# colmap/glomap

Hardware: NVIDIA H100
Metric: observations/sec per BA LM-iteration (higher is better)
Workload: dtype f64

## Files before the change

### glomap_b200/csrc/ba_kernels.cuh

```cuda
#pragma once
#include "common.cuh"
#include "pcg.cuh"

namespace b200 {

constexpr int kCamRec = 8;
constexpr int kIntrRec = 8;
constexpr double kZEps = 1e-12;
constexpr int kSeg = 256;
__host__ __device__ constexpr int seg_split(int n) { return n <= 0 ? 0 : (n < kSeg + kSeg / 2 ? 1 : (n + kSeg / 2) / kSeg); }
constexpr int kIntrSmem = 16;
constexpr int kJpDoubles = 6;
constexpr int kSensorRec = 16;

struct BAView {
  int C, P, K;
  long long N;
  int n_tiles;
  int n_segs;
  int min_views;
  const int* obs_cam;
  const int* obs_pt;
  const double2* obs_xy;
  const unsigned* pt_begin;
// ... 401 lines not shown
      sm.red[5][tid] = o.Jp[2] * o.Jp[2] + o.Jp[5] * o.Jp[5];
      sm.red[6][tid] = o.Jp[0] * o.r[0] + o.Jp[3] * o.r[1];
      sm.red[7][tid] = o.Jp[1] * o.r[0] + o.Jp[4] * o.r[1];
      sm.red[8][tid] = o.Jp[2] * o.r[0] + o.Jp[5] * o.r[1];
      fence_proxy_async_smem();
      __syncthreads();
      if (tid == 0) {
        if (V2) tma_store_1d(v.W + (size_t)(o0 + c0) * kJpDoubles, sm.Wt, (uint32_t)nc * kJpDoubles * 8);
        else tma_store_1d(v.W + (size_t)(o0 + c0) * kWDoubles, sm.Wt, (uint32_t)nc * kWBytes);
        tma_store_commit();
      }
      for (int item = tid; item < npts * 9; item += kTile) {
        const int j = item / 9, k = item - 9 * j;
        const int lo = max((int)sm.pb[j] - (int)(o0 + c0), 0), hi = min((int)sm.pb[j + 1] - (int)(o0 + c0), nc);
        double a = 0.0;
        for (int i = lo; i < hi; ++i) a += sm.red[k][i];
        sm.acc[k][j] += a;
      }
      if (tid == 0) tma_store_wait_read();
      __syncthreads();
    }
  }
  double gmax = 0.0;
  if (points_var && tid < npts) {
    const size_t p = (size_t)(p0 + tid);
    if (pvalid) {
#pragma unroll
      for (int k = 0; k < 6; ++k) v.V[6 * p + k] = sm.acc[k][tid];
#pragma unroll
      for (int k = 0; k < 3; ++k) {
        const double gk = sm.acc[6 + k][tid];
        v.gp[3 * p + k] = gk;
        gmax = fmax(gmax, fabs(gk));
      }
    } else {
#pragma unroll
      for (int k = 0; k < 6; ++k) v.V[6 * p + k] = 0.0;
#pragma unroll
      for (int k = 0; k < 3; ++k) v.gp[3 * p + k] = 0.0;
    }
  }
  cost = block_sum(cost, sm.scratch);
  if (tid == 0 && cost != 0.0) atomicAdd(&scal[0], cost);
  gmax = block_max(gmax, sm.scratch);
  if (tid == 0 && gmax > 0.0) atomic_max_nonneg(&scal[1], gmax);
}

__global__ void __launch_bounds__(128) ba_linearize_cams(BAView v, const double* __restrict__ cam_rec,
                                                        const double* __restrict__ intr_rec,
                                                        const double* __restrict__ points, double huber_a) {
  const int warp = (blockIdx.x * blockDim.x + threadIdx.x) >> 5;
  const int lane = threadIdx.x & 31;
  if (warp >= v.n_segs) return;
  const int cam = v.seg_cam[warp];
  const int b = v.seg_begin[warp], e = v.seg_end[warp];
  const double4 q4c = *reinterpret_cast<const double4*>(cam_rec + (size_t)cam * kCamRec);
  const double4 t4c = *reinterpret_cast<const double4*>(cam_rec + (size_t)cam * kCamRec + 4);
  const double* irc = intr_rec + (size_t)v.seg_intr[warp] * kIntrRec;
  const double* src = sensor_of_seg(v, warp);
  double U[21], g[6];
#pragma unroll
  for (int k = 0; k < 21; ++k) U[k] = 0.0;
#pragma unroll
  for (int k = 0; k < 6; ++k) g[k] = 0.0;
  for (int i = b + lane; i < e; i += 32) {
    const int pt = v.pt_c[i];
    const double2 xy = v.xy_c[i];
    const double X0 = points[3 * (size_t)pt], X1 = points[3 * (size_t)pt + 1], X2 = points[3 * (size_t)pt + 2];
    ObsLin o;
    linearize_obs(q4c, t4c, irc, src, X0, X1, X2, xy, huber_a, o);
    double Jc[2][6];
#pragma unroll
    for (int a = 0; a < 2; ++a)
#pragma unroll
      for (int k = 0; k < 3; ++k) {
        Jc[a][k] = o.Jr[3 * a + k];
        Jc[a][3 + k] = o.Jt[3 * a + k];
      }
    int idx = 0;
#pragma unroll
    for (int i2 = 0; i2 < 6; ++i2) {
#pragma unroll
      for (int j = i2; j < 6; ++j) U[idx++] += Jc[0][i2] * Jc[0][j] + Jc[1][i2] * Jc[1][j];
      g[i2] += Jc[0][i2] * o.r[0] + Jc[1][i2] * o.r[1];
    }
  }
#pragma unroll
  for (int k = 0; k < 21; ++k) {
    const double s = warp_sum(U[k]);
    if (lane == k && s != 0.0) atomicAdd(&v.U[(size_t)cam * 21 + k], s);
  }
#pragma unroll
  for (int k = 0; k < 6; ++k) {
    const double s = warp_sum(g[k]);
    if (lane == 21 + k && s != 0.0) atomicAdd(&v.gc[(size_t)cam * 6 + k], s);
  }
}

__global__ void ba_finalize_cams(int C, double* __restrict__ U, double* __restrict__ gc,
                                 const unsigned char* __restrict__ cam_mask, double* __restrict__ jscale_c,
                                 int set_jscale, double* __restrict__ scal, const double* __restrict__ gslots, int nslots) {
  const int c = blockIdx.x * blockDim.x + threadIdx.x;
  double gmax = 0.0;
  if (blockIdx.x == 0 && threadIdx.x < nslots) gmax = gslots[threadIdx.x];
  if (c < C) {
    const int mask = cam_mask[c];
#pragma unroll
    for (int i = 0; i < 6; ++i) {
      const int di = sym_idx(6, i, i);
      const bool fixed = (i < 3) ? (mask & 1) : (mask & 2);
      double d = U[(size_t)c * 21 + di];
      if (fixed || !(d > 0.0)) {
        for (int j = 0; j < 6; ++j) U[(size_t)c * 21 + (i <= j ? sym_idx(6, i, j) : sym_idx(6, j, i))] = 0.0;
        U[(size_t)c * 21 + di] = 1.0;
        gc[(size_t)c * 6 + i] = 0.0;
        if (set_jscale) jscale_c[(size_t)c * 6 + i] = -1.0;
      } else {
        if (set_jscale) jscale_c[(size_t)c * 6 + i] = 1.0 / (1.0 + sqrt(d));
        gmax = fmax(gmax, fabs(gc[(size_t)c * 6 + i]));
      }
    }
  }
  gmax = warp_max(gmax);
  if ((threadIdx.x & 31) == 0 && gmax > 0.0) atomic_max_nonneg(&scal[1], gmax);
}

__global__ void ba_damp_cams(int C, const double* __restrict__ U, const double* __restrict__ jscale_c, double radius,
                             double* __restrict__ Dc) {
  const int i = blockIdx.x * blockDim.x + threadIdx.x;
  if (i >= C * 6) return;
  const int c = i / 6, k = i % 6;
  const double js = jscale_c[i];
  if (js < 0.0) {
    Dc[i] = 0.0;
    return;
  }
  const double d = U[(size_t)c * 21 + sym_idx(6, k, k)];
  const double js2 = js * js;
  Dc[i] = fmin(fmax(d * js2, 1e-6), 1e32) / (radius * js2);
}

__device__ __forceinline__ void point_damping(const double* V6, const double* js, double radius, double Dp[3]) {
  const double d[3] = {V6[0], V6[3], V6[5]};
#pragma unroll
  for (int k = 0; k < 3; ++k) {
    const double js2 = js[k] * js[k];
    Dp[k] = fmin(fmax(d[k] * js2, 1e-6), 1e32) / (radius * js2);
  }
}
__global__ void ba_damp_points(int P, const double* __restrict__ V, double* __restrict__ jscale_p, int set_jscale,
                               double radius, double* __restrict__ Vinv) {
  const int p = blockIdx.x * blockDim.x + threadIdx.x;
  if (p >= P) return;
  double v6[6];
#pragma unroll
  for (int k = 0; k < 6; ++k) v6[k] = V[6 * (size_t)p + k];
  double js[3];
  if (set_jscale) {
    js[0] = 1.0 / (1.0 + sqrt(v6[0]));
    js[1] = 1.0 / (1.0 + sqrt(v6[3]));
    js[2] = 1.0 / (1.0 + sqrt(v6[5]));
#pragma unroll
    for (int k = 0; k < 3; ++k) jscale_p[3 * (size_t)p + k] = js[k];
  } else {
#pragma unroll
    for (int k = 0; k < 3; ++k) js[k] = jscale_p[3 * (size_t)p + k];
  }
  double Dp[3];
  point_damping(v6, js, radius, Dp);
  v6[0] += Dp[0];
  v6[3] += Dp[1];
  v6[5] += Dp[2];
  double inv[6];
  sym3_inverse(v6, inv);
#pragma unroll
  for (int k = 0; k < 6; ++k) Vinv[6 * (size_t)p + k] = inv[k];
}

__global__ void __launch_bounds__(128) ba_schur_diag(BAView v) {
  const int warp = (blockIdx.x * blockDim.x + threadIdx.x) >> 5;
  const int lane = threadIdx.x & 31;
  if (warp >= v.n_segs) return;
  const int cam = v.seg_cam[warp];
  const int b = v.seg_begin[warp], e = v.seg_end[warp];
  double S[21];
#pragma unroll
  for (int k = 0; k < 21; ++k) S[k] = 0.0;
  for (int i = b + lane; i < e; i += 32) {
    const int o = v.camord_obs[i];
    const int pt = v.pt_c[i];
    double w[18], vi[6];
    const double2* wp = reinterpret_cast<const double2*>(v.W + (size_t)o * kWDoubles);
#pragma unroll
    for (int k = 0; k < 9; ++k) {
      const double2 t = wp[k];
      w[2 * k] = t.x;
      w[2 * k + 1] = t.y;
    }
    const double2* vp = reinterpret_cast<const double2*>(v.Vinv + (size_t)pt * 6);
#pragma unroll
    for (int k = 0; k < 3; ++k) {
      const double2 t = vp[k];
      vi[2 * k] = t.x;
      vi[2 * k + 1] = t.y;
    }
    double T[6][3];
#pragma unroll
    for (int r = 0; r < 6; ++r) sym3_mul(vi, &w[3 * r], T[r]);
    int idx = 0;
#pragma unroll
    for (int r = 0; r < 6; ++r)
#pragma unroll
      for (int c = r; c < 6; ++c)
        S[idx++] += T[r][0] * w[3 * c] + T[r][1] * w[3 * c + 1] + T[r][2] * w[3 * c + 2];
  }
#pragma unroll
  for (int k = 0; k < 21; ++k) {
    const double s = warp_sum(S[k]);
    if (lane == k && s != 0.0) atomicAdd(&v.Sd[(size_t)cam * 21 + k], s);
  }
}

__global__ void ba_build_precond(int C, const double* __restrict__ U, const double* __restrict__ Dc,
                                 const double* __restrict__ Sd, double* __restrict__ Minv) {
  const int c = blockIdx.x * blockDim.x + threadIdx.x;
  if (c >= C) return;
  double m[21];
#pragma unroll
  for (int k = 0; k < 21; ++k) m[k] = U[(size_t)c * 21 + k] - (Sd ? Sd[(size_t)c * 21 + k] : 0.0);
#pragma unroll
  for (int i = 0; i < 6; ++i) m[sym_idx(6, i, i)] += Dc[(size_t)c * 6 + i];
  double inv[21];
  spd_inverse_packed<6>(m, inv);
#pragma unroll
  for (int k = 0; k < 21; ++k) Minv[(size_t)c * 21 + k] = inv[k];
}

struct K3Smem {
  alignas(128) double Wt[kTile * kWDoubles];
  double t[3][kTile + 1];
  double z[3][kTilePts + 1];
  unsigned pb[kTilePts + 1];
  double scratch[32];
  alignas(8) uint64_t mbar;
};

template <int MODE>
__global__ void __launch_bounds__(kTile, B200_K3_MIN_CTAS) ba_schur_pass(BAView v, const double* __restrict__ x, double* __restrict__ y,
                                                          const double* __restrict__ points,
                                                          double* __restrict__ points_new, double radius,
                                                          double* __restrict__ bscal, const double* __restrict__ spk = nullptr,
                                                          const double* __restrict__ dk = nullptr, int m_intr = 0,
                                                          const PcgCtl* __restrict__ ctl = nullptr) {
  extern __shared__ __align__(128) unsigned char smem_raw[];
  if (ctl && ctl->done) return;
  K3Smem& sm = *reinterpret_cast<K3Smem*>(smem_raw);
  const int tile = blockIdx.x;
  const int tid = threadIdx.x;
  const int4 td = v.tile_desc[tile];
  const int p0 = td.x, npts = td.y, n = td.w;
  const unsigned o0 = (unsigned)td.z, o1 = o0 + (unsigned)n;
  const int nchunks = (n + kTile - 1) / kTile;
  if (tid == 0) {
    mbar_init(&sm.mbar, 1);
    fence_mbar_init();
    if (MODE != 1 && n > 0) {
      const int nc0 = min(kTile, n);
      mbar_arrive_expect_tx(&sm.mbar, (uint32_t)nc0 * kWBytes);
      tma_load_1d(sm.Wt, v.W + (size_t)o0 * kWDoubles, (uint32_t)nc0 * kWBytes, &sm.mbar);
    }
  }
  int cam_pf = 0, pt_pf = 0;
  double2 xa_pf = make_double2(0, 0), xb_pf = xa_pf, xc_pf = xa_pf;
  if (MODE != 1 && tid < n) {
    cam_pf = v.obs_cam[o0 + tid];
    if (MODE == 0) pt_pf = v.obs_pt[o0 + tid];
    const double2* xp = reinterpret_cast<const double2*>(x + (size_t)cam_pf * 6);
    xa_pf = xp[0];
    xb_pf = xp[1];
    xc_pf = xp[2];
  }
  if (tid < npts) {
    sm.pb[tid] = v.pt_begin[p0 + tid];
    if (tid == npts - 1) sm.pb[npts] = o1;
    sm.z[0][tid] = sm.z[1][tid] = sm.z[2][tid] = 0.0;
  }
  __syncthreads();
  uint32_t phase = 0;
  if (MODE != 1) {
    for (int ch = 0; ch < nchunks; ++ch) {
      const int c0 = ch * kTile;
      const int nc = min(kTile, n - c0);
      if (tid == 0 && ch > 0) {
        mbar_arrive_expect_tx(&sm.mbar, (uint32_t)nc * kWBytes);
        tma_load_1d(sm.Wt, v.W + (size_t)(o0 + c0) * kWDoubles, (uint32_t)nc * kWBytes, &sm.mbar);
      }
      double xc[6] = {0, 0, 0, 0, 0, 0};
      const bool active = tid < nc;
      if (active) {
        if (ch > 0) {
          cam_pf = v.obs_cam[o0 + c0 + tid];
          const double2* xp = reinterpret_cast<const double2*>(x + (size_t)cam_pf * 6);
          xa_pf = xp[0];
          xb_pf = xp[1];
          xc_pf = xp[2];
        }
        xc[0] = xa_pf.x; xc[1] = xa_pf.y; xc[2] = xb_pf.x; xc[3] = xb_pf.y; xc[4] = xc_pf.x; xc[5] = xc_pf.y;
      }
      mbar_wait(&sm.mbar, phase);
      phase ^= 1;
      double t0 = 0, t1 = 0, t2 = 0;
      if (active) {
        const double2* wr = reinterpret_cast<const double2*>(sm.Wt + tid * kWDoubles);
#pragma unroll
        for (int r = 0; r < 6; r += 2) {
          const double2 q0 = wr[(3 * r) / 2], q1 = wr[(3 * r) / 2 + 1], q2 = wr[(3 * r) / 2 + 2];
          t0 += q0.x * xc[r] + q1.y * xc[r + 1];
          t1 += q0.y * xc[r] + q2.x * xc[r + 1];
          t2 += q1.x * xc[r] + q2.y * xc[r + 1];
        }
      }
      sm.t[0][tid] = t0;
      sm.t[1][tid] = t1;
      sm.t[2][tid] = t2;
      __syncthreads();
      for (int item = tid; item < npts * 3; item += kTile) {
        const int j = item / 3, k = item - 3 * j;
        const int lo = max((int)sm.pb[j] - (int)(o0 + c0), 0), hi = min((int)sm.pb[j + 1] - (int)(o0 + c0), nc);
        double a = 0.0;
// ... 254 lines not shown
```

### glomap_b200/csrc/ba_kernels_v3.cuh

```cuda
#pragma once
#include "ba_kernels_v2.cuh"

namespace b200 {

constexpr int kEllWindow = 1024;
constexpr int kEllThreads = 128;

struct EllView {
  int n_groups;
  const int* row0;
  const int* pt;
  const int* len;
  const int* cam;
  const double2* xy;
  const unsigned short* sensor;
  double* A;
  double* B = nullptr;
};

template <class Sort>
__global__ void __launch_bounds__(kEllWindow) ell_sort_window(int P, int min_views, const unsigned* __restrict__ pt_begin,
                                                              int* __restrict__ ell_pt, int* __restrict__ ell_len,
                                                              int* __restrict__ ell_slot, int* __restrict__ group_rows) {
  __shared__ typename Sort::TempStorage tmp;
  const int t = threadIdx.x;
  const int p = blockIdx.x * kEllWindow + t;
  int len = -1;
  if (p < P) {
    len = (int)(pt_begin[p + 1] - pt_begin[p]);
    if (len < min_views) len = 0;
  }
  unsigned key[1] = {p < P ? (unsigned)(0xffffff - min(len, 0xffffff)) : 0xffffffffu};
  int val[1] = {t};
  Sort(tmp).Sort(key, val, 0, 25);
  const int src = blockIdx.x * kEllWindow + val[0];
  const int slot = blockIdx.x * kEllWindow + t;
  const bool real = key[0] != 0xffffffffu;
  const int l = real ? (int)(0xffffff - key[0]) : 0;
  ell_pt[slot] = real ? src : -1;
  ell_len[slot] = l;
  if (real) ell_slot[src] = slot;
  if ((t & 31) == 0) group_rows[slot >> 5] = l;
}

__global__ void ell_scatter_obs(long long N, int min_views, const int* __restrict__ obs_pt, const unsigned* __restrict__ pt_begin,
                                const int* __restrict__ obs_cam, const double2* __restrict__ obs_xy,
                                const unsigned short* __restrict__ obs_sensor, const int* __restrict__ ell_slot,
                                const int* __restrict__ row0, int* __restrict__ ell_cam, double2* __restrict__ ell_xy,
                                unsigned short* __restrict__ ell_sensor) {
  const long long o = (long long)blockIdx.x * blockDim.x + threadIdx.x;
  if (o >= N) return;
  const int p = obs_pt[o];
  const unsigned b = pt_begin[p];
  if ((int)(pt_begin[p + 1] - b) < min_views) return;
  const int slot = ell_slot[p];
  const size_t dst = ((size_t)row0[slot >> 5] + (size_t)(o - b)) * 32 + (slot & 31);
  ell_cam[dst] = obs_cam[o];
  ell_xy[dst] = obs_xy[o];
  if (obs_sensor) ell_sensor[dst] = obs_sensor[o];
}

template <int NK>
__global__ void __launch_bounds__(kEllThreads, NK > 0 ? 3 : B200_E1_MIN_CTAS) ba3_linearize_points(BAView v, EllView ell,
                                                                               const double* __restrict__ cam_rec,
                                                                               const double* __restrict__ intr_rec,
                                                                               const double* __restrict__ points,
                                                                               double huber_a, int points_var,
                                                                               double* __restrict__ part_cost,
                                                                               double* __restrict__ part_gmax,
                                                                               const IntrVarRec* __restrict__ ivar) {
  const int slot = blockIdx.x * kEllThreads + threadIdx.x;
  const int lane = threadIdx.x & 31;
  const int g = slot >> 5;
  double cost = 0.0, gmax = 0.0;
  if (g < ell.n_groups) {
    const int pt = ell.pt[slot];
    const int mylen = ell.len[slot];
    const int r0 = ell.row0[g], nrow = ell.row0[g + 1] - r0;
    double X0 = 0, X1 = 0, X2 = 0;
    if (pt >= 0) {
      X0 = points[3 * (size_t)pt]; X1 = points[3 * (size_t)pt + 1]; X2 = points[3 * (size_t)pt + 2];
    }
    double V[6] = {0, 0, 0, 0, 0, 0}, gp[3] = {0, 0, 0};
#if B200_E1_PIPE
    int camB = 0;
    double2 xyA = make_double2(0, 0), xyB = xyA;
    double4 qA = make_double4(0, 0, 0, 1), tA = make_double4(0, 0, 0, 0);
    if (mylen > 0) {
      const size_t i0 = (size_t)r0 * 32 + lane;
      const int camA = ld_stream(ell.cam + i0);
      xyA = ld_stream(ell.xy + i0);
      if (mylen > 1) {
        camB = ld_stream(ell.cam + i0 + 32);
        xyB = ld_stream(ell.xy + i0 + 32);
      }
      qA = ld_rec32(cam_rec + (size_t)camA * kCamRec);
      tA = ld_rec32(cam_rec + (size_t)camA * kCamRec + 4);
    }
#if B200_E1_PIPE >= 2
    double4 qB2 = qA, tB2 = tA;
    int camC2 = 0;
    if (mylen > 1) {
      qB2 = ld_rec32(cam_rec + (size_t)camB * kCamRec);
      tB2 = ld_rec32(cam_rec + (size_t)camB * kCamRec + 4);
    }
    if (mylen > 2) camC2 = ld_stream(ell.cam + (size_t)r0 * 32 + lane + 64);
#endif
    for (int j = 0; j < nrow; ++j) {
      if (j >= mylen) break;
      const size_t idx = ((size_t)r0 + j) * 32 + lane;
#if B200_E1_PIPE >= 2
      double4 qB = qB2, tB = tB2;
      double4 qC = qB2, tC = tB2;
      int camC = 0, camD = 0;
      double2 xyC = xyB;
      if (j + 2 < mylen) {
        qC = ld_rec32(cam_rec + (size_t)camC2 * kCamRec);
        tC = ld_rec32(cam_rec + (size_t)camC2 * kCamRec + 4);
        xyC = ld_stream(ell.xy + idx + 64);
      }
      if (j + 3 < mylen) camD = ld_stream(ell.cam + idx + 96);
      (void)camC;
#else
      double4 qB = qA, tB = tA;
      int camC = 0;
      double2 xyC = xyB;
      if (j + 1 < mylen) {
        qB = ld_rec32(cam_rec + (size_t)camB * kCamRec);
        tB = ld_rec32(cam_rec + (size_t)camB * kCamRec + 4);
      }
      if (j + 2 < mylen) {
        camC = ld_stream(ell.cam + idx + 64);
        xyC = ld_stream(ell.xy + idx + 64);
      }
#endif
      const double* sr = ell.sensor ? v.sensor_rec + (size_t)ell.sensor[idx] * kSensorRec : nullptr;
      const int blk = obs_intr_idx(tA, sr);
      const double* ir = intr_rec + (size_t)blk * kIntrRec;
      ObsCore o;
      obs_core(qA, tA, ir, sr, X0, X1, X2, xyA, huber_a, o);
      cost += 0.5 * o.rho0;
      if (points_var) {
        double Jp[6], A[6], b[3];
        obs_point_blocks(o, Jp, A, b);
        double* row = ell.A + ((size_t)r0 + j) * (6 * 32) + lane;
#pragma unroll
        for (int k = 0; k < 6; ++k) {
          st_stream(row + 32 * k, A[k]);
          V[k] += A[k];
        }
        gp[0] += b[0]; gp[1] += b[1]; gp[2] += b[2];
        if (NK > 0) {
          constexpr int NKK = NK > 0 ? NK : 1;
          double Jk[2][NKK], Bo[3 * NKK];
          obs_intr_rows<NK>(o, ld_intr(ir), ivar[blk], Jp, Jk, Bo);
          double* rowB = ell.B + ((size_t)r0 + j) * (3 * NK * 32) + lane;
#pragma unroll
          for (int k = 0; k < 3 * NK; ++k) st_stream(rowB + 32 * k, Bo[k]);
        }
      }
#if B200_E1_PIPE >= 2
      qA = qB; tA = tB; qB2 = qC; tB2 = tC; xyA = xyB; xyB = xyC; camC2 = camD;
#else
      qA = qB; tA = tB; xyA = xyB; xyB = xyC; camB = camC;
#endif
    }
#else
#pragma unroll 2
    for (int j = 0; j < nrow; ++j) {
      if (j >= mylen) continue;
      const size_t idx = ((size_t)r0 + j) * 32 + lane;
      const int cam = ld_stream(ell.cam + idx);
      const double2 xy = ld_stream(ell.xy + idx);
      const double4 q4 = ld_rec32(cam_rec + (size_t)cam * kCamRec);
      const double4 t4 = ld_rec32(cam_rec + (size_t)cam * kCamRec + 4);
      const double* sr = ell.sensor ? v.sensor_rec + (size_t)ell.sensor[idx] * kSensorRec : nullptr;
      const int blk = obs_intr_idx(t4, sr);
      const double* ir = intr_rec + (size_t)blk * kIntrRec;
      ObsCore o;
      obs_core(q4, t4, ir, sr, X0, X1, X2, xy, huber_a, o);
      cost += 0.5 * o.rho0;
      if (points_var) {
        double Jp[6], A[6], b[3];
        obs_point_blocks(o, Jp, A, b);
        double* row = ell.A + ((size_t)r0 + j) * (6 * 32) + lane;
#pragma unroll
        for (int k = 0; k < 6; ++k) {
          st_stream(row + 32 * k, A[k]);
          V[k] += A[k];
        }
        gp[0] += b[0]; gp[1] += b[1]; gp[2] += b[2];
        if (NK > 0) {
          constexpr int NKK = NK > 0 ? NK : 1;
          double Jk[2][NKK], Bo[3 * NKK];
          obs_intr_rows<NK>(o, ld_intr(ir), ivar[blk], Jp, Jk, Bo);
          double* rowB = ell.B + ((size_t)r0 + j) * (3 * NK * 32) + lane;
#pragma unroll
          for (int k = 0; k < 3 * NK; ++k) st_stream(rowB + 32 * k, Bo[k]);
        }
      }
    }
#endif
    if (points_var && pt >= 0) {
#pragma unroll
      for (int k = 0; k < 6; ++k) v.V[6 * (size_t)pt + k] = V[k];
#pragma unroll
      for (int k = 0; k < 3; ++k) {
        v.gp[3 * (size_t)pt + k] = gp[k];
        gmax = fmax(gmax, fabs(gp[k]));
      }
    }
  }
  cost = warp_sum(cost);
  gmax = warp_max(gmax);
  if (lane == 0) {
    part_cost[slot >> 5] = cost;
    part_gmax[slot >> 5] = gmax;
  }
}

__global__ void __launch_bounds__(kEllThreads) ba3_cost(BAView v, EllView ell, const double* __restrict__ cam_rec,
                                                         const double* __restrict__ intr_rec,
                                                         const double* __restrict__ points, double huber_a,
                                                         double* __restrict__ part_cost) {
  __shared__ double scratch[32];
  const int slot = blockIdx.x * kEllThreads + threadIdx.x;
  const int lane = threadIdx.x & 31;
  const int g = slot >> 5;
  double cost = 0.0;
  if (g < ell.n_groups) {
    const int pt = ell.pt[slot];
    const int mylen = ell.len[slot];
    const int r0 = ell.row0[g], nrow = ell.row0[g + 1] - r0;
    double X0 = 0, X1 = 0, X2 = 0;
    if (pt >= 0) {
      X0 = points[3 * (size_t)pt]; X1 = points[3 * (size_t)pt + 1]; X2 = points[3 * (size_t)pt + 2];
    }
#pragma unroll 2
    for (int j = 0; j < nrow; ++j) {
      if (j >= mylen) continue;
      const size_t idx = ((size_t)r0 + j) * 32 + lane;
      const int cam = ld_stream(ell.cam + idx);
      const double2 xy = ld_stream(ell.xy + idx);
      const double4 q4 = ld_rec32(cam_rec + (size_t)cam * kCamRec);
      const double4 t4 = ld_rec32(cam_rec + (size_t)cam * kCamRec + 4);
      const double* sr = ell.sensor ? v.sensor_rec + (size_t)ell.sensor[idx] * kSensorRec : nullptr;
      const double* ir = intr_rec + (size_t)obs_intr_idx(t4, sr) * kIntrRec;
      const double q[4] = {q4.x, q4.y, q4.z, q4.w};
      double R[9];
      quat_to_R(q, R);
      double xc = R[0] * X0 + R[1] * X1 + R[2] * X2 + t4.x;
      double yc = R[3] * X0 + R[4] * X1 + R[5] * X2 + t4.y;
      double zc = R[6] * X0 + R[7] * X1 + R[8] * X2 + t4.z;
      if (sr) sensor_apply(sr, xc, yc, zc);
      if (zc > kZEps) {
        double px, py;
        project_only(ir, xc, yc, zc, px, py);
        const double e0 = px - xy.x, e1 = py - xy.y;
        double rho0, rho1;
        huber(e0 * e0 + e1 * e1, huber_a, rho0, rho1);
        cost += 0.5 * rho0;
      }
    }
  }
  cost = block_sum(cost, scratch);
  if (threadIdx.x == 0) part_cost[blockIdx.x] = cost;
}

__global__ void __launch_bounds__(1024) ba3_reduce_partials(int n, const double* __restrict__ part_a,
                                                           const double* __restrict__ part_b, double* __restrict__ out_sum,
                                                           double* __restrict__ out_max) {
  __shared__ double scratch[32];
  double s = 0.0, m = 0.0;
  for (int i = threadIdx.x; i < n; i += blockDim.x) {
    s += part_a[i];
    if (part_b) m = fmax(m, part_b[i]);
  }
  s = block_sum(s, scratch);
  if (threadIdx.x == 0) *out_sum = s;
  if (part_b) {
    m = block_max(m, scratch);
    if (threadIdx.x == 0) *out_max = m;
  }
}

template <int MODE, int NK>
__global__ void __launch_bounds__(kEllThreads, MODE == 0 ? B200_EA_MIN_CTAS : B200_EA2_MIN_CTAS) ba3_pass_a(
    BAView v, EllView ell, BAViewV2 v2, const double* __restrict__ xp, const double* __restrict__ points,
    double* __restrict__ points_new, double radius, double* __restrict__ bscal, const PcgCtl* __restrict__ ctl) {
  __shared__ double scratch[32];
  if (ctl && ctl->done) return;
  const int slot = blockIdx.x * kEllThreads + threadIdx.x;
  const int lane = threadIdx.x & 31;
  const int g = slot >> 5;
  double b0 = 0, b1 = 0, b2 = 0, b3 = 0;
  if (g < ell.n_groups) {
    const int pt = ell.pt[slot];
    const int mylen = ell.len[slot];
    const int r0 = ell.row0[g], nrow = ell.row0[g + 1] - r0;
    double X0 = 0, X1 = 0, X2 = 0;
    if (pt >= 0) {
      X0 = points[3 * (size_t)pt]; X1 = points[3 * (size_t)pt + 1]; X2 = points[3 * (size_t)pt + 2];
    }
    double s0 = 0, s1 = 0, s2 = 0;
#pragma unroll 4
    for (int j = 0; j < nrow; ++j) {
      if (j >= mylen) continue;
      const size_t idx = ((size_t)r0 + j) * 32 + lane;
      const int cam = ld_stream(ell.cam + idx);
      const double* row = ell.A + ((size_t)r0 + j) * (6 * 32) + lane;
      const double a0 = ld_stream(row), a1 = ld_stream(row + 32), a2 = ld_stream(row + 64);
      const double a3 = ld_stream(row + 96), a4 = ld_stream(row + 128), a5 = ld_stream(row + 160);
      double xr0, xr1, xr2, xt0;
      ld_nc_256(xp + (size_t)cam * kXqStride, xr0, xr1, xr2, xt0);
      double4 xt;
      if (NK > 0) {
        xt = ld_rec32(xp + (size_t)cam * kXqStride + 4);
      } else {
        const double2 xt12 = __ldg(reinterpret_cast<const double2*>(xp + (size_t)cam * kXqStride + 4));
        xt = make_double4(xt12.x, xt12.y, 0.0, 0.0);
      }
      const double w0 = xt0 - 2.0 * (X1 * xr2 - X2 * xr1);
      const double w1 = xt.x - 2.0 * (X2 * xr0 - X0 * xr2);
      const double w2 = xt.y - 2.0 * (X0 * xr1 - X1 * xr0);
      s0 += a0 * w0 + a1 * w1 + a2 * w2;
      s1 += a1 * w0 + a3 * w1 + a4 * w2;
      s2 += a2 * w0 + a4 * w1 + a5 * w2;
      if (NK > 0) {
        const double* rowB = ell.B + ((size_t)r0 + j) * (3 * NK * 32) + lane;
        const double xk[2] = {xt.z, xt.w};
#pragma unroll
        for (int k = 0; k < NK; ++k) {
          s0 += ld_stream(rowB + 32 * (3 * k)) * xk[k];
          s1 += ld_stream(rowB + 32 * (3 * k + 1)) * xk[k];
          s2 += ld_stream(rowB + 32 * (3 * k + 2)) * xk[k];
        }
      }
    }
    if (pt >= 0) {
      const size_t p = (size_t)pt;
      double z[3] = {0.0, 0.0, 0.0};
      if (mylen > 0) {
        double s[3] = {s0, s1, s2};
        double gq[3] = {0, 0, 0};
        if (MODE != 0) {
          gq[0] = v.gp[3 * p]; gq[1] = v.gp[3 * p + 1]; gq[2] = v.gp[3 * p + 2];
          s[0] += gq[0]; s[1] += gq[1]; s[2] += gq[2];
        }
        const double2* vp = reinterpret_cast<const double2*>(v.Vinv + 6 * p);
        const double2 va = vp[0], vb = vp[1], vc = vp[2];
        const double vi[6] = {va.x, va.y, vb.x, vb.y, vc.x, vc.y};
        sym3_mul(vi, s, z);
        if (MODE == 2) {
          double v6[6], js[3], Dp[3];
#pragma unroll
          for (int k = 0; k < 6; ++k) v6[k] = v.V[6 * p + k];
#pragma unroll
          for (int k = 0; k < 3; ++k) js[k] = v.jscale_p[3 * p + k];
          point_damping(v6, js, radius, Dp);
          const double Xo[3] = {X0, X1, X2};
#pragma unroll
          for (int k = 0; k < 3; ++k) {
            const double dp = -z[k];
            points_new[3 * p + k] = Xo[k] + dp;
            b0 += gq[k] * dp;
            b1 += Dp[k] * dp * dp;
            b2 += dp * dp;
            b3 += Xo[k] * Xo[k];
          }
        }
      } else if (MODE == 2) {
        points_new[3 * p] = X0; points_new[3 * p + 1] = X1; points_new[3 * p + 2] = X2;
      }
      if (MODE == 0) st_keep4(v2.z4 + 4 * p, make_double4(z[0], z[1], z[2], 0.0), l2_policy_evict_last());
    }
  }
  if (MODE == 2) {
    b0 = block_sum(b0, scratch);
    b1 = block_sum(b1, scratch);
    b2 = block_sum(b2, scratch);
    b3 = block_sum(b3, scratch);
    if (threadIdx.x == 0) {
      double* o = bscal + (size_t)blockIdx.x * 4;
      o[0] = b0; o[1] = b1; o[2] = b2; o[3] = b3;
    }
  }
}

}
```

### glomap_b200/csrc/common.cuh

```cuda
#pragma once
#include <cuda_runtime.h>
#include <stdint.h>
#include <stdio.h>

#include <string>

namespace b200 {

#ifndef B200_TILE
#define B200_TILE 128
#endif
#ifndef B200_K1_MIN_CTAS
#define B200_K1_MIN_CTAS 5
#endif
#ifndef B200_K3_MIN_CTAS
#define B200_K3_MIN_CTAS 8
#endif
#ifndef B200_PA_MIN_CTAS
#define B200_PA_MIN_CTAS 12
#endif
#ifndef B200_LC_MIN_CTAS
#define B200_LC_MIN_CTAS 3
#endif
#ifndef B200_PB_MIN_CTAS
#define B200_PB_MIN_CTAS 4
#endif
#ifndef B200_SD_MIN_CTAS
#define B200_SD_MIN_CTAS 3
#endif
#ifndef B200_E1_MIN_CTAS
#define B200_E1_MIN_CTAS 4
#endif
#ifndef B200_E1_PIPE
#define B200_E1_PIPE 1
#endif
#ifndef B200_EA_MIN_CTAS
#define B200_EA_MIN_CTAS 8
#endif
#ifndef B200_EA2_MIN_CTAS
#define B200_EA2_MIN_CTAS 6
#endif
#ifndef B200_STREAM_HINTS
#define B200_STREAM_HINTS 1
#endif
constexpr int kTile = B200_TILE;
constexpr int kTilePts = 64;
constexpr int kWDoubles = 18;
constexpr int kWBytes = kWDoubles * 8;

#define B200_CUDA_OK(expr)                                                                     \
  do {                                                                                         \
    cudaError_t err__ = (expr);                                                                \
    if (err__ != cudaSuccess) {                                                                \
      throw ::b200::CudaError(std::string(#expr) + ": " + cudaGetErrorString(err__), __LINE__); \
    }                                                                                          \
  } while (0)

struct CudaError {
  std::string msg;
  int line;
  CudaError(std::string m, int l) : msg(std::move(m)), line(l) {}
};
struct InvalidInput {
  std::string msg;
};

__device__ __forceinline__ uint32_t smem_u32(const void* p) { return (uint32_t)__cvta_generic_to_shared(p); }

__device__ __forceinline__ void mbar_init(uint64_t* bar, int count) {
  asm volatile("mbarrier.init.shared::cta.b64 [%0], %1;" ::"r"(smem_u32(bar)), "r"(count));
}
__device__ __forceinline__ void fence_mbar_init() { asm volatile("fence.mbarrier_init.release.cluster;" ::: "memory"); }
__device__ __forceinline__ void fence_proxy_async_smem() { asm volatile("fence.proxy.async.shared::cta;" ::: "memory"); }

__device__ __forceinline__ void mbar_arrive_expect_tx(uint64_t* bar, uint32_t bytes) {
  asm volatile("mbarrier.arrive.expect_tx.shared::cta.b64 _, [%0], %1;" ::"r"(smem_u32(bar)), "r"(bytes) : "memory");
}
__device__ __forceinline__ void mbar_wait(uint64_t* bar, uint32_t parity) {
  asm volatile(
      "{\n"
      ".reg .pred p;\n"
      "WAIT_LOOP:\n"
      "mbarrier.try_wait.parity.shared::cta.b64 p, [%0], %1;\n"
      "@p bra WAIT_DONE;\n"
      "bra WAIT_LOOP;\n"
      "WAIT_DONE:\n"
      "}\n" ::"r"(smem_u32(bar)),
      "r"(parity)
      : "memory");
}
__device__ __forceinline__ void tma_load_1d(void* smem_dst, const void* gsrc, uint32_t bytes, uint64_t* bar) {
  asm volatile("cp.async.bulk.shared::cluster.global.mbarrier::complete_tx::bytes [%0], [%1], %2, [%3];" ::"r"(
                   smem_u32(smem_dst)),
               "l"(gsrc), "r"(bytes), "r"(smem_u32(bar))
               : "memory");
}
__device__ __forceinline__ uint64_t l2_policy_evict_first() {
  uint64_t p;
  asm volatile("createpolicy.fractional.L2::evict_first.b64 %0, 1.0;" : "=l"(p));
  return p;
}
__device__ __forceinline__ void tma_load_1d_stream(void* smem_dst, const void* gsrc, uint32_t bytes, uint64_t* bar) {
#if B200_STREAM_HINTS
  const uint64_t pol = l2_policy_evict_first();
  asm volatile(
      "cp.async.bulk.shared::cluster.global.mbarrier::complete_tx::bytes.L2::cache_hint [%0], [%1], %2, [%3], %4;" ::"r"(
          smem_u32(smem_dst)),
      "l"(gsrc), "r"(bytes), "r"(smem_u32(bar)), "l"(pol)
      : "memory");
#else
  tma_load_1d(smem_dst, gsrc, bytes, bar);
#endif
}
__device__ __forceinline__ void prefetch_l1(const void* p) { asm volatile("prefetch.global.L1 [%0];" ::"l"(p)); }
__device__ __forceinline__ void ld_nc_256(const double* p, double& a, double& b, double& c, double& d) {
  asm volatile("ld.global.nc.v2.f64 {%0, %1}, [%2];" : "=d"(a), "=d"(b) : "l"(p));
  asm volatile("ld.global.nc.v2.f64 {%0, %1}, [%2];" : "=d"(c), "=d"(d) : "l"(p + 2));
}
#ifndef B200_REC_CG
#define B200_REC_CG 0
#endif
__device__ __forceinline__ double4 ld_rec32(const double* p) {
  double4 r;
#if B200_REC_CG
  asm("ld.global.cg.v2.f64 {%0, %1}, [%2];" : "=d"(r.x), "=d"(r.y) : "l"(p));
  asm("ld.global.cg.v2.f64 {%0, %1}, [%2];" : "=d"(r.z), "=d"(r.w) : "l"(p + 2));
#else
  asm("ld.global.nc.v2.f64 {%0, %1}, [%2];" : "=d"(r.x), "=d"(r.y) : "l"(p));
  asm("ld.global.nc.v2.f64 {%0, %1}, [%2];" : "=d"(r.z), "=d"(r.w) : "l"(p + 2));
#endif
  return r;
}
__device__ __forceinline__ void st_rec32(double* p, double a, double b, double c, double d) {
  asm volatile("st.global.v2.f64 [%0], {%1, %2};" ::"l"(p), "d"(a), "d"(b) : "memory");
  asm volatile("st.global.v2.f64 [%0], {%1, %2};" ::"l"(p + 2), "d"(c), "d"(d) : "memory");
}
template <class T>
__device__ __forceinline__ T ld_stream(const T* p) {
#if B200_STREAM_HINTS
  return __ldcs(p);
#else
  return *p;
#endif
}
template <class T>
__device__ __forceinline__ void st_stream(T* p, T v) {
#if B200_STREAM_HINTS
  __stcs(p, v);
#else
  *p = v;
#endif
}
#ifndef B200_KEEP_HINTS
#define B200_KEEP_HINTS 0
#endif
__device__ __forceinline__ uint64_t l2_policy_evict_last() {
  uint64_t p;
  asm volatile("createpolicy.fractional.L2::evict_last.b64 %0, 1.0;" : "=l"(p));
  return p;
}
__device__ __forceinline__ double4 ld_keep4(const double* p, uint64_t pol) {
#if B200_KEEP_HINTS
  double4 v;
  asm volatile("ld.global.L2::cache_hint.v2.f64 {%0, %1}, [%2], %3;" : "=d"(v.x), "=d"(v.y) : "l"(p), "l"(pol));
  asm volatile("ld.global.L2::cache_hint.v2.f64 {%0, %1}, [%2], %3;" : "=d"(v.z), "=d"(v.w) : "l"(p + 2), "l"(pol));
  return v;
#else
  return ld_rec32(p);
#endif
}
__device__ __forceinline__ void st_keep4(double* p, double4 v, uint64_t pol) {
#if B200_KEEP_HINTS
  asm volatile("st.global.L2::cache_hint.v2.f64 [%0], {%1, %2}, %3;" ::"l"(p), "d"(v.x), "d"(v.y), "l"(pol) : "memory");
  asm volatile("st.global.L2::cache_hint.v2.f64 [%0], {%1, %2}, %3;" ::"l"(p + 2), "d"(v.z), "d"(v.w), "l"(pol) : "memory");
#else
  st_rec32(p, v.x, v.y, v.z, v.w);
#endif
}
__device__ __forceinline__ void tma_store_1d(void* gdst, const void* smem_src, uint32_t bytes) {
  asm volatile("cp.async.bulk.global.shared::cta.bulk_group [%0], [%1], %2;" ::"l"(gdst), "r"(smem_u32(smem_src)),
               "r"(bytes)
               : "memory");
}
__device__ __forceinline__ void tma_store_commit() { asm volatile("cp.async.bulk.commit_group;" ::: "memory"); }
__device__ __forceinline__ void tma_store_wait_read() { asm volatile("cp.async.bulk.wait_group.read 0;" ::: "memory"); }
__device__ __forceinline__ void tma_store_wait_all() { asm volatile("cp.async.bulk.wait_group 0;" ::: "memory"); }

// ... 169 lines not shown
```

### profiles/kernel_times.py

```python
#!/usr/bin/env python
import argparse
import collections
import os
import sys

ROOT = os.path.dirname(os.path.dirname(os.path.abspath(__file__)))
sys.path.insert(0, ROOT)


def main():
    ap = argparse.ArgumentParser()
    ap.add_argument("--workload", default="config4")
    ap.add_argument("--optimize-intrinsics", type=int, default=0)
    ap.add_argument("--solves", type=int, default=2)
    ap.add_argument("--top", type=int, default=14)
    args = ap.parse_args()
    import torch
    from bench import WORKLOADS
    from glomap_b200 import estimators as E, synthetic as S

    C, P, L, chunk = WORKLOADS[args.workload]
    sc = S.make_scene(C, P, L, seed=1, pixel_sigma=0.5, chunk=chunk, point_range=(0, P))
    init = S.perturb_scene(sc, chunk=chunk, point_offset=0)
    mask = E.first_frame_mask(C)
    torch.cuda.set_device(0)
    ctx = E.Context(0, 0, 1, None)
    opts = E.BundleAdjusterOptions(optimize_intrinsics=bool(args.optimize_intrinsics))
    opts.solver_options.max_num_iterations = 20
    opts.solver_options.pcg_rel_tolerance = 0.05
    opts.solver_options.pcg_max_iterations = 200
    torch.cuda.synchronize()
    free0 = torch.cuda.mem_get_info()[0]
    prob = E.BAProblem(ctx, sc, 3, mask)
    prob.set_state(init.intr_params, init.quat, init.trans, init.points)
    prob.save_state()
    prob.solve(opts)
    torch.cuda.synchronize()
    free1 = torch.cuda.mem_get_info()[0]
    its = []
    with torch.profiler.profile(activities=[torch.profiler.ProfilerActivity.CUDA]) as prof:
        for _ in range(args.solves):
            prob.restore_state()
            st = prob.solve(opts).as_dict()
            its.append((st["iterations"], st["pcg_iterations"]))
        torch.cuda.synchronize()
    agg = collections.defaultdict(lambda: [0, 0.0])
    for ev in prof.events():
        if ev.device_type == torch.autograd.DeviceType.CUDA and ev.name and not ev.name.startswith("Memcpy") \
                and not ev.name.startswith("Memset"):
            name = ev.name.split("(")[0].replace("void ", "").replace("b200::", "")
            agg[name][0] += 1
            agg[name][1] += ev.device_time_total
    tot = sum(v[1] for v in agg.values())
    print(f"{args.workload} optimize_intrinsics={args.optimize_intrinsics} env="
          f"{ {k: v for k, v in os.environ.items() if k.startswith('B200SFM_')} } LM/PCG per solve {its}")
    print(f"device memory held by the resident problem after one solve: {(free0 - free1) / 1e9:.3f} GB")
    print("| kernel | launches | total ms | avg us |\n|---|---|---|---|")
    for k, (n, us) in sorted(agg.items(), key=lambda kv: -kv[1][1])[:args.top]:
        print(f"| `{k}` | {n} | {us / 1e3:.3f} | {us / n:.1f} |")
    print(f"total kernel time {tot / 1e3 / args.solves:.2f} ms per solve\n")
    prob.free()
    ctx.close()


if __name__ == "__main__":
    main()
```

Measured before the change: 1.593 billion.

## Gather camera records cooperatively via shuffles and shared-memory transpose in ELL linearize/cost

Replaces per-lane 64-byte camera record loads in the ELL point linearization (NK==0) and cost kernels with a warp-cooperative gather. Four lanes each fetch a 16-byte slice of a camera record, and the results are transposed through padded shared memory, with a one-row-ahead prefetch. This aims to coalesce the random camera gathers into fewer, fuller memory transactions, at the cost of shared memory, warp syncs and shuffles. It also vectorizes the 6-double V loads and stores to double2, batches the partial-sum reduction loads, drops the B200_E1_PIPE variants, and adds wall-clock and idle-gap reporting to the profiling script.

After: 1.620 billion, median of 6. +1.7%, better.

```diff
diff --git a/glomap_b200/csrc/ba_kernels.cuh b/glomap_b200/csrc/ba_kernels.cuh
--- a/glomap_b200/csrc/ba_kernels.cuh
+++ b/glomap_b200/csrc/ba_kernels.cuh
@@ -577,9 +577,9 @@
                                double radius, double* __restrict__ Vinv) {
   const int p = blockIdx.x * blockDim.x + threadIdx.x;
   if (p >= P) return;
-  double v6[6];
-#pragma unroll
-  for (int k = 0; k < 6; ++k) v6[k] = V[6 * (size_t)p + k];
+  const double2* vr = reinterpret_cast<const double2*>(V + 6 * (size_t)p);
+  const double2 va = vr[0], vb = vr[1], vc = vr[2];
+  double v6[6] = {va.x, va.y, vb.x, vb.y, vc.x, vc.y};
   double js[3];
   if (set_jscale) {
     js[0] = 1.0 / (1.0 + sqrt(v6[0]));
@@ -598,8 +598,10 @@
   v6[5] += Dp[2];
   double inv[6];
   sym3_inverse(v6, inv);
-#pragma unroll
-  for (int k = 0; k < 6; ++k) Vinv[6 * (size_t)p + k] = inv[k];
+  double2* vo = reinterpret_cast<double2*>(Vinv + 6 * (size_t)p);
+  vo[0] = make_double2(inv[0], inv[1]);
+  vo[1] = make_double2(inv[2], inv[3]);
+  vo[2] = make_double2(inv[4], inv[5]);
 }
 
 __global__ void __launch_bounds__(128) ba_schur_diag(BAView v) {
diff --git a/glomap_b200/csrc/ba_kernels_v3.cuh b/glomap_b200/csrc/ba_kernels_v3.cuh
--- a/glomap_b200/csrc/ba_kernels_v3.cuh
+++ b/glomap_b200/csrc/ba_kernels_v3.cuh
@@ -60,6 +60,26 @@
   if (obs_sensor) ell_sensor[dst] = obs_sensor[o];
 }
 
+constexpr int kCamStage = 5;
+__device__ __forceinline__ void cam_gather_issue(const double* __restrict__ cam_rec, int cam, int lane, double2 v[4]) {
+#pragma unroll
+  for (int r = 0; r < 4; ++r) {
+    const int c = __shfl_sync(0xffffffffu, cam, 8 * r + (lane >> 2));
+    v[r] = c >= 0 ? __ldg(reinterpret_cast<const double2*>(cam_rec + (size_t)c * kCamRec) + (lane & 3)) : make_double2(0, 0);
+  }
+}
+__device__ __forceinline__ void cam_gather_finish(double2* __restrict__ stage, int lane, const double2 v[4], double4& q4,
+                                                  double4& t4) {
+  __syncwarp();
+#pragma unroll
+  for (int r = 0; r < 4; ++r) stage[(8 * r + (lane >> 2)) * kCamStage + (lane & 3)] = v[r];
+  __syncwarp();
+  const double2* s = stage + lane * kCamStage;
+  const double2 a = s[0], b = s[1], c = s[2], d = s[3];
+  q4 = make_double4(a.x, a.y, b.x, b.y);
+  t4 = make_double4(c.x, c.y, d.x, d.y);
+}
+
 template <int NK>
 __global__ void __launch_bounds__(kEllThreads, NK > 0 ? 3 : B200_E1_MIN_CTAS) ba3_linearize_points(BAView v, EllView ell,
                                                                                const double* __restrict__ cam_rec,
@@ -69,6 +89,7 @@
                                                                                double* __restrict__ part_cost,
                                                                                double* __restrict__ part_gmax,
                                                                                const IntrVarRec* __restrict__ ivar) {
+  __shared__ double2 stage_all[NK == 0 ? kEllThreads * kCamStage : 1];
   const int slot = blockIdx.x * kEllThreads + threadIdx.x;
   const int lane = threadIdx.x & 31;
   const int g = slot >> 5;
@@ -82,98 +103,7 @@
       X0 = points[3 * (size_t)pt]; X1 = points[3 * (size_t)pt + 1]; X2 = points[3 * (size_t)pt + 2];
     }
     double V[6] = {0, 0, 0, 0, 0, 0}, gp[3] = {0, 0, 0};
-#if B200_E1_PIPE
-    int camB = 0;
-    double2 xyA = make_double2(0, 0), xyB = xyA;
-    double4 qA = make_double4(0, 0, 0, 1), tA = make_double4(0, 0, 0, 0);
-    if (mylen > 0) {
-      const size_t i0 = (size_t)r0 * 32 + lane;
-      const int camA = ld_stream(ell.cam + i0);
-      xyA = ld_stream(ell.xy + i0);
-      if (mylen > 1) {
-        camB = ld_stream(ell.cam + i0 + 32);
-        xyB = ld_stream(ell.xy + i0 + 32);
-      }
-      qA = ld_rec32(cam_rec + (size_t)camA * kCamRec);
-      tA = ld_rec32(cam_rec + (size_t)camA * kCamRec + 4);
-    }
-#if B200_E1_PIPE >= 2
-    double4 qB2 = qA, tB2 = tA;
-    int camC2 = 0;
-    if (mylen > 1) {
-      qB2 = ld_rec32(cam_rec + (size_t)camB * kCamRec);
-      tB2 = ld_rec32(cam_rec + (size_t)camB * kCamRec + 4);
-    }
-    if (mylen > 2) camC2 = ld_stream(ell.cam + (size_t)r0 * 32 + lane + 64);
-#endif
-    for (int j = 0; j < nrow; ++j) {
-      if (j >= mylen) break;
-      const size_t idx = ((size_t)r0 + j) * 32 + lane;
-#if B200_E1_PIPE >= 2
-      double4 qB = qB2, tB = tB2;
-      double4 qC = qB2, tC = tB2;
-      int camC = 0, camD = 0;
-      double2 xyC = xyB;
-      if (j + 2 < mylen) {
-        qC = ld_rec32(cam_rec + (size_t)camC2 * kCamRec);
-        tC = ld_rec32(cam_rec + (size_t)camC2 * kCamRec + 4);
-        xyC = ld_stream(ell.xy + idx + 64);
-      }
-      if (j + 3 < mylen) camD = ld_stream(ell.cam + idx + 96);
-      (void)camC;
-#else
-      double4 qB = qA, tB = tA;
-      int camC = 0;
-      double2 xyC = xyB;
-      if (j + 1 < mylen) {
-        qB = ld_rec32(cam_rec + (size_t)camB * kCamRec);
-        tB = ld_rec32(cam_rec + (size_t)camB * kCamRec + 4);
-      }
-      if (j + 2 < mylen) {
-        camC = ld_stream(ell.cam + idx + 64);
-        xyC = ld_stream(ell.xy + idx + 64);
-      }
-#endif
-      const double* sr = ell.sensor ? v.sensor_rec + (size_t)ell.sensor[idx] * kSensorRec : nullptr;
-      const int blk = obs_intr_idx(tA, sr);
-      const double* ir = intr_rec + (size_t)blk * kIntrRec;
-      ObsCore o;
-      obs_core(qA, tA, ir, sr, X0, X1, X2, xyA, huber_a, o);
-      cost += 0.5 * o.rho0;
-      if (points_var) {
-        double Jp[6], A[6], b[3];
-        obs_point_blocks(o, Jp, A, b);
-        double* row = ell.A + ((size_t)r0 + j) * (6 * 32) + lane;
-#pragma unroll
-        for (int k = 0; k < 6; ++k) {
-          st_stream(row + 32 * k, A[k]);
-          V[k] += A[k];
-        }
-        gp[0] += b[0]; gp[1] += b[1]; gp[2] += b[2];
-        if (NK > 0) {
-          constexpr int NKK = NK > 0 ? NK : 1;
-          double Jk[2][NKK], Bo[3 * NKK];
-          obs_intr_rows<NK>(o, ld_intr(ir), ivar[blk], Jp, Jk, Bo);
-          double* rowB = ell.B + ((size_t)r0 + j) * (3 * NK * 32) + lane;
-#pragma unroll
-          for (int k = 0; k < 3 * NK; ++k) st_stream(rowB + 32 * k, Bo[k]);
-        }
-      }
-#if B200_E1_PIPE >= 2
-      qA = qB; tA = tB; qB2 = qC; tB2 = tC; xyA = xyB; xyB = xyC; camC2 = camD;
-#else
-      qA = qB; tA = tB; xyA = xyB; xyB = xyC; camB = camC;
-#endif
-    }
-#else
-#pragma unroll 2
-    for (int j = 0; j < nrow; ++j) {
-      if (j >= mylen) continue;
-      const size_t idx = ((size_t)r0 + j) * 32 + lane;
-      const int cam = ld_stream(ell.cam + idx);
-      const double2 xy = ld_stream(ell.xy + idx);
-      const double4 q4 = ld_rec32(cam_rec + (size_t)cam * kCamRec);
-      const double4 t4 = ld_rec32(cam_rec + (size_t)cam * kCamRec + 4);
+    auto observe = [&](int j, size_t idx, const double4& q4, const double4& t4, double2 xy) {
       const double* sr = ell.sensor ? v.sensor_rec + (size_t)ell.sensor[idx] * kSensorRec : nullptr;
       const int blk = obs_intr_idx(t4, sr);
       const double* ir = intr_rec + (size_t)blk * kIntrRec;
@@ -199,11 +129,65 @@
           for (int k = 0; k < 3 * NK; ++k) st_stream(rowB + 32 * k, Bo[k]);
         }
       }
-    }
-#endif
+    };
+    int camA = -1, camB = -1;
+    double2 xyA = make_double2(0, 0), xyB = xyA;
+    const size_t i0 = (size_t)r0 * 32 + lane;
+    if (mylen > 0) {
+      camA = ld_stream(ell.cam + i0);
+      xyA = ld_stream(ell.xy + i0);
+    }
+    if (mylen > 1) {
+      camB = ld_stream(ell.cam + i0 + 32);
+      xyB = ld_stream(ell.xy + i0 + 32);
+    }
+    if constexpr (NK == 0) {
+      double2* stage = stage_all + (threadIdx.x & ~31) * kCamStage;
+      double2 recA[4];
+      cam_gather_issue(cam_rec, camA, lane, recA);
+      for (int j = 0; j < nrow; ++j) {
+        const size_t idx = ((size_t)r0 + j) * 32 + lane;
+        double4 qA, tA;
+        cam_gather_finish(stage, lane, recA, qA, tA);
+        cam_gather_issue(cam_rec, camB, lane, recA);
+        int camC = -1;
+        double2 xyC = xyB;
+        if (j + 2 < mylen) {
+          camC = ld_stream(ell.cam + idx + 64);
+          xyC = ld_stream(ell.xy + idx + 64);
+        }
+        if (j < mylen) observe(j, idx, qA, tA, xyA);
+        xyA = xyB; xyB = xyC; camB = camC;
+      }
+    } else {
+      double4 qA = make_double4(0, 0, 0, 1), tA = make_double4(0, 0, 0, 0);
+      if (mylen > 0) {
+        qA = ld_rec32(cam_rec + (size_t)camA * kCamRec);
+        tA = ld_rec32(cam_rec + (size_t)camA * kCamRec + 4);
+      }
+      for (int j = 0; j < nrow; ++j) {
+        if (j >= mylen) break;
+        const size_t idx = ((size_t)r0 + j) * 32 + lane;
+        double4 qB = qA, tB = tA;
+        int camC = 0;
+        double2 xyC = xyB;
+        if (j + 1 < mylen) {
+          qB = ld_rec32(cam_rec + (size_t)camB * kCamRec);
+          tB = ld_rec32(cam_rec + (size_t)camB * kCamRec + 4);
+        }
+        if (j + 2 < mylen) {
+          camC = ld_stream(ell.cam + idx + 64);
+          xyC = ld_stream(ell.xy + idx + 64);
+        }
+        observe(j, idx, qA, tA, xyA);
+        qA = qB; tA = tB; xyA = xyB; xyB = xyC; camB = camC;
+      }
+    }
     if (points_var && pt >= 0) {
-#pragma unroll
-      for (int k = 0; k < 6; ++k) v.V[6 * (size_t)pt + k] = V[k];
+      double2* vo = reinterpret_cast<double2*>(v.V + 6 * (size_t)pt);
+      vo[0] = make_double2(V[0], V[1]);
+      vo[1] = make_double2(V[2], V[3]);
+      vo[2] = make_double2(V[4], V[5]);
 #pragma unroll
       for (int k = 0; k < 3; ++k) {
         v.gp[3 * (size_t)pt + k] = gp[k];
@@ -224,9 +208,11 @@
                                                          const double* __restrict__ points, double huber_a,
                                                          double* __restrict__ part_cost) {
   __shared__ double scratch[32];
+  __shared__ double2 stage_all[kEllThreads * kCamStage];
   const int slot = blockIdx.x * kEllThreads + threadIdx.x;
   const int lane = threadIdx.x & 31;
   const int g = slot >> 5;
+  double2* stage = stage_all + (threadIdx.x & ~31) * kCamStage;
   double cost = 0.0;
   if (g < ell.n_groups) {
     const int pt = ell.pt[slot];
@@ -236,31 +222,50 @@
     if (pt >= 0) {
       X0 = points[3 * (size_t)pt]; X1 = points[3 * (size_t)pt + 1]; X2 = points[3 * (size_t)pt + 2];
     }
-#pragma unroll 2
+    int camA = -1, camB = -1;
+    double2 xyA = make_double2(0, 0), xyB = xyA;
+    const size_t i0 = (size_t)r0 * 32 + lane;
+    if (mylen > 0) {
+      camA = ld_stream(ell.cam + i0);
+      xyA = ld_stream(ell.xy + i0);
+    }
+    if (mylen > 1) {
+      camB = ld_stream(ell.cam + i0 + 32);
+      xyB = ld_stream(ell.xy + i0 + 32);
+    }
+    double2 recA[4];
+    cam_gather_issue(cam_rec, camA, lane, recA);
     for (int j = 0; j < nrow; ++j) {
-      if (j >= mylen) continue;
       const size_t idx = ((size_t)r0 + j) * 32 + lane;
-      const int cam = ld_stream(ell.cam + idx);
-      const double2 xy = ld_stream(ell.xy + idx);
-      const double4 q4 = ld_rec32(cam_rec + (size_t)cam * kCamRec);
-      const double4 t4 = ld_rec32(cam_rec + (size_t)cam * kCamRec + 4);
-      const double* sr = ell.sensor ? v.sensor_rec + (size_t)ell.sensor[idx] * kSensorRec : nullptr;
-      const double* ir = intr_rec + (size_t)obs_intr_idx(t4, sr) * kIntrRec;
-      const double q[4] = {q4.x, q4.y, q4.z, q4.w};
-      double R[9];
-      quat_to_R(q, R);
-      double xc = R[0] * X0 + R[1] * X1 + R[2] * X2 + t4.x;
-      double yc = R[3] * X0 + R[4] * X1 + R[5] * X2 + t4.y;
-      double zc = R[6] * X0 + R[7] * X1 + R[8] * X2 + t4.z;
-      if (sr) sensor_apply(sr, xc, yc, zc);
-      if (zc > kZEps) {
-        double px, py;
-        project_only(ir, xc, yc, zc, px, py);
-        const double e0 = px - xy.x, e1 = py - xy.y;
-        double rho0, rho1;
-        huber(e0 * e0 + e1 * e1, huber_a, rho0, rho1);
-        cost += 0.5 * rho0;
-      }
+      double4 q4, t4;
+      cam_gather_finish(stage, lane, recA, q4, t4);
+      cam_gather_issue(cam_rec, camB, lane, recA);
+      int camC = -1;
+      double2 xyC = xyB;
+      if (j + 2 < mylen) {
+        camC = ld_stream(ell.cam + idx + 64);
+        xyC = ld_stream(ell.xy + idx + 64);
+      }
+      if (j < mylen) {
+        const double* sr = ell.sensor ? v.sensor_rec + (size_t)ell.sensor[idx] * kSensorRec : nullptr;
+        const double* ir = intr_rec + (size_t)obs_intr_idx(t4, sr) * kIntrRec;
+        const double q[4] = {q4.x, q4.y, q4.z, q4.w};
+        double R[9];
+        quat_to_R(q, R);
+        double xc = R[0] * X0 + R[1] * X1 + R[2] * X2 + t4.x;
+        double yc = R[3] * X0 + R[4] * X1 + R[5] * X2 + t4.y;
+        double zc = R[6] * X0 + R[7] * X1 + R[8] * X2 + t4.z;
+        if (sr) sensor_apply(sr, xc, yc, zc);
+        if (zc > kZEps) {
+          double px, py;
+          project_only(ir, xc, yc, zc, px, py);
+          const double e0 = px - xyA.x, e1 = py - xyA.y;
+          double rho0, rho1;
+          huber(e0 * e0 + e1 * e1, huber_a, rho0, rho1);
+          cost += 0.5 * rho0;
+        }
+      }
+      xyA = xyB; xyB = xyC; camB = camC;
     }
   }
   cost = block_sum(cost, scratch);
@@ -272,7 +277,22 @@
                                                            double* __restrict__ out_max) {
   __shared__ double scratch[32];
   double s = 0.0, m = 0.0;
-  for (int i = threadIdx.x; i < n; i += blockDim.x) {
+  constexpr int kBatch = 8;
+  int i = threadIdx.x;
+  for (; i + (kBatch - 1) * (int)blockDim.x < n; i += kBatch * blockDim.x) {
+    double a[kBatch], b[kBatch];
+#pragma unroll
+    for (int k = 0; k < kBatch; ++k) {
+      a[k] = part_a[i + k * blockDim.x];
+      b[k] = part_b ? part_b[i + k * blockDim.x] : 0.0;
+    }
+#pragma unroll
+    for (int k = 0; k < kBatch; ++k) {
+      s += a[k];
+      if (part_b) m = fmax(m, b[k]);
+    }
+  }
+  for (; i < n; i += blockDim.x) {
     s += part_a[i];
     if (part_b) m = fmax(m, part_b[i]);
   }
@@ -353,8 +373,9 @@
         sym3_mul(vi, s, z);
         if (MODE == 2) {
           double v6[6], js[3], Dp[3];
-#pragma unroll
-          for (int k = 0; k < 6; ++k) v6[k] = v.V[6 * p + k];
+          const double2* vr = reinterpret_cast<const double2*>(v.V + 6 * p);
+          const double2 v01 = vr[0], v23 = vr[1], v45 = vr[2];
+          v6[0] = v01.x; v6[1] = v01.y; v6[2] = v23.x; v6[3] = v23.y; v6[4] = v45.x; v6[5] = v45.y;
 #pragma unroll
           for (int k = 0; k < 3; ++k) js[k] = v.jscale_p[3 * p + k];
           point_damping(v6, js, radius, Dp);
diff --git a/glomap_b200/csrc/common.cuh b/glomap_b200/csrc/common.cuh
--- a/glomap_b200/csrc/common.cuh
+++ b/glomap_b200/csrc/common.cuh
@@ -30,9 +30,6 @@
 #endif
 #ifndef B200_E1_MIN_CTAS
 #define B200_E1_MIN_CTAS 4
-#endif
-#ifndef B200_E1_PIPE
-#define B200_E1_PIPE 1
 #endif
 #ifndef B200_EA_MIN_CTAS
 #define B200_EA_MIN_CTAS 8
diff --git a/profiles/kernel_times.py b/profiles/kernel_times.py
--- a/profiles/kernel_times.py
+++ b/profiles/kernel_times.py
@@ -37,6 +37,16 @@
     prob.solve(opts)
     torch.cuda.synchronize()
     free1 = torch.cuda.mem_get_info()[0]
+    wall = []
+    for _ in range(args.solves):
+        prob.restore_state()
+        torch.cuda.synchronize()
+        e0, e1 = torch.cuda.Event(enable_timing=True), torch.cuda.Event(enable_timing=True)
+        e0.record()
+        prob.solve(opts)
+        e1.record()
+        torch.cuda.synchronize()
+        wall.append(e0.elapsed_time(e1))
     its = []
     with torch.profiler.profile(activities=[torch.profiler.ProfilerActivity.CUDA]) as prof:
         for _ in range(args.solves):
@@ -45,12 +55,14 @@
             its.append((st["iterations"], st["pcg_iterations"]))
         torch.cuda.synchronize()
     agg = collections.defaultdict(lambda: [0, 0.0])
+    timeline = []
     for ev in prof.events():
-        if ev.device_type == torch.autograd.DeviceType.CUDA and ev.name and not ev.name.startswith("Memcpy") \
-                and not ev.name.startswith("Memset"):
+        if ev.device_type == torch.autograd.DeviceType.CUDA and ev.name:
             name = ev.name.split("(")[0].replace("void ", "").replace("b200::", "")
-            agg[name][0] += 1
-            agg[name][1] += ev.device_time_total
+            timeline.append((ev.time_range.start, ev.time_range.end, name))
+            if not ev.name.startswith("Memcpy") and not ev.name.startswith("Memset"):
+                agg[name][0] += 1
+                agg[name][1] += ev.device_time_total
     tot = sum(v[1] for v in agg.values())
     print(f"{args.workload} optimize_intrinsics={args.optimize_intrinsics} env="
           f"{ {k: v for k, v in os.environ.items() if k.startswith('B200SFM_')} } LM/PCG per solve {its}")
@@ -59,6 +71,25 @@
     for k, (n, us) in sorted(agg.items(), key=lambda kv: -kv[1][1])[:args.top]:
         print(f"| `{k}` | {n} | {us / 1e3:.3f} | {us / n:.1f} |")
     print(f"total kernel time {tot / 1e3 / args.solves:.2f} ms per solve\n")
+    timeline.sort()
+    gap = collections.defaultdict(lambda: [0, 0.0])
+    busy_end = timeline[0][1] if timeline else 0.0
+    for st, en, name in timeline[1:]:
+        if st > busy_end:
+            gap[name][0] += 1
+            gap[name][1] += st - busy_end
+        busy_end = max(busy_end, en)
+    wall.sort()
+    med = wall[len(wall) // 2]
+    idle = sum(v[1] for v in gap.values())
+    print(f"step budget: solve {med:.2f} ms (CUDA events, profiler off, median of {len(wall)}: "
+          f"{' / '.join(f'{w:.2f}' for w in wall)}), kernels {tot / 1e3 / args.solves:.2f} ms, "
+          f"difference {med - tot / 1e3 / args.solves:.2f} ms; idle between device activities in the trace "
+          f"{idle / 1e3 / args.solves:.2f} ms per solve")
+    print("| idle before | gaps | total ms per solve | avg us |\n|---|---|---|---|")
+    for k, (n, us) in sorted(gap.items(), key=lambda kv: -kv[1][1])[:args.top]:
+        print(f"| `{k}` | {n // args.solves} | {us / 1e3 / args.solves:.3f} | {us / n:.1f} |")
+    print()
     prob.free()
     ctx.close()
 
```
